# OpenDriveLab/ViDAR

Measured on AMD Instinct MI355X. Metric: train samples/sec (6-cam->BEV step), higher is better.
Workload: dtype f32

## Files before the change

vidar_amd/csrc/gemm_mfma.hip:

```cpp
#include <hip/hip_runtime.h>

#include <stdint.h>

#include <type_traits>

#include "vidar_hip.h"
#include "vidar_common.h"

namespace {

typedef __bf16 bf16x8 __attribute__((ext_vector_type(8)));
typedef __bf16 bf16x2 __attribute__((ext_vector_type(2)));
typedef float f32x16 __attribute__((ext_vector_type(16)));
typedef float f32x2 __attribute__((ext_vector_type(2)));
typedef float f32x4 __attribute__((ext_vector_type(4)));
typedef float f32x4u __attribute__((ext_vector_type(4), aligned(4)));
typedef uint32_t u32x4 __attribute__((ext_vector_type(4)));
typedef uint32_t u32x2 __attribute__((ext_vector_type(2)));

constexpr int BM = 128, BN = 128, THREADS = 256;
constexpr int BK = 32;
constexpr int MN_STRIDE = 128 + 8;
template <int PREC>
struct Geo {
  static constexpr int UNITS = (PREC == 1) ? 16 : 32;
  static constexpr int KM_STRIDE = (PREC == 1) ? UNITS : UNITS + 4;
  static constexpr int IMG_DWORDS = (128 * KM_STRIDE > UNITS * MN_STRIDE) ? 128 * KM_STRIDE : UNITS * MN_STRIDE;
  static constexpr int NS = UNITS / 8;
};
constexpr int PREC_F32 = 0, PREC_BF16X3 = 1;
constexpr int LAY_K = 0, LAY_MN = 1;

struct GemmArgs {
  const float* A; const float* B; float* C;
  int64_t lda, ldb, ldc, sA, sB, sC;
  int M, N, K;
  int splits, k_chunk;
  int slabs;
  const float* scale; const float* shift; int vec_axis;
  const float* residual; int64_t ldr, sR;
  int relu;
  int tiles_m, tiles_n, m_fastest;
  int total;
  float* a_rowsum;
  float* rowsum_ws;
};

struct Lane {
  int wm, wn, l31, h;
  __device__ __forceinline__ Lane(int tid, int wave) : wm((wave >> 1) * 64), wn((wave & 1) * 64), l31(tid & 31), h((tid & 63) >> 5) {}
  __device__ __forceinline__ explicit Lane(int tid) : Lane(tid, tid >> 6) {}
  __device__ __forceinline__ uint32_t voff(uint32_t ld) const { return (uint32_t)(((wm + 4 * h) * ld + wn + l31) * 4); }
};

__device__ __forceinline__ void zero_acc(f32x16 (&acc)[2][2]) {
#pragma unroll
  for (int i = 0; i < 2; ++i)
#pragma unroll
    for (int j = 0; j < 2; ++j)
#pragma unroll
      for (int r = 0; r < 16; ++r) acc[i][j][r] = 0.0f;
}

struct Staged {
  static constexpr int CH = 2;
  f32x4 v[CH][2];
};

constexpr int KM_LPR = 8;
constexpr int KM_RPI = 64 / KM_LPR;
constexpr int KM_NI = 32 / KM_RPI;

__device__ __forceinline__ __amdgpu_buffer_rsrc_t make_rsrc(const float* p, int64_t bytes = 0x7fffffff) {
  const uint64_t a = (uint64_t)p;
  const uint32_t lo = __builtin_amdgcn_readfirstlane((uint32_t)a), hi = __builtin_amdgcn_readfirstlane((uint32_t)(a >> 32));
  const int32_t n = __builtin_amdgcn_readfirstlane((int32_t)(bytes > 0x7fffffff ? 0x7fffffff : bytes));
  return __builtin_amdgcn_make_buffer_rsrc((void*)(((uint64_t)hi << 32) | lo), 0, n, 0x00020000);
}
__device__ __forceinline__ __amdgpu_buffer_rsrc_t window_rsrc(const float* base, int64_t ld, int rows_left, int cols_left,
                                                              bool present = true) {
  return make_rsrc(base, present ? ((int64_t)(rows_left - 1) * ld + cols_left) * 4 : 0);
}
__device__ __forceinline__ f32x4 ld16(__amdgpu_buffer_rsrc_t r, uint32_t voff, uint32_t soff) {
  return __builtin_bit_cast(f32x4, __builtin_amdgcn_raw_buffer_load_b128(r, voff, soff, 0));
}
__device__ __forceinline__ float ld4(__amdgpu_buffer_rsrc_t r, uint32_t voff, uint32_t soff) {
  return __builtin_bit_cast(float, __builtin_amdgcn_raw_buffer_load_b32(r, voff, soff, 0));
}

template <int PREC, int LAY>
__device__ __forceinline__ uint32_t voff(int64_t ld, int tid) {
  if (LAY == LAY_K) {
    const int lane = tid & 63, wave = tid >> 6;
    return (uint32_t)(((32 * wave + lane / KM_LPR) * (uint32_t)ld + (lane % KM_LPR) * 4) * 4);
  }
  const int kr = (PREC == PREC_BF16X3) ? (tid >> 5) * 2 : (tid >> 5);
  return (uint32_t)((kr * (uint32_t)ld + (tid & 31) * 4) * 4);
}

template <int PREC, int LAY>
__device__ __forceinline__ void load(Staged& s, __amdgpu_buffer_rsrc_t rs, int64_t ld, int krel, int k0, int kend, int tid,
                                     uint32_t vo) {
  if (LAY == LAY_K) {
#pragma unroll
    for (int i = 0; i < KM_NI; ++i)
      s.v[i >> 1][i & 1] = ld16(rs, vo, (uint32_t)((i * KM_RPI * (uint32_t)ld + krel) * 4));
    const bool tail = k0 + BK > kend;
    if (tail) {
      const int k = k0 + ((tid & 63) % KM_LPR) * 4;
#pragma unroll
      for (int i = 0; i < KM_NI; ++i)
#pragma unroll
        for (int j = 0; j < 4; ++j) s.v[i >> 1][i & 1][j] = (k + j < kend) ? s.v[i >> 1][i & 1][j] : 0.0f;
    }
  } else {
#pragma unroll
    for (int i = 0; i < Staged::CH * 2; ++i) {
      const int ku = (PREC == PREC_BF16X3) ? 16 * (i >> 1) + (i & 1) : 8 * i;
      s.v[i >> 1][i & 1] = ld16(rs, vo, (uint32_t)(krel + ku) * (uint32_t)ld * 4u);
    }
  }
}

__device__ __forceinline__ void split2(float a, float b, uint32_t& hi, uint32_t& lo) {
  f32x2 x = {a, b};
  bf16x2 h = __builtin_convertvector(x, bf16x2);
  f32x2 r = x - __builtin_convertvector(h, f32x2);
  bf16x2 l = __builtin_convertvector(r, bf16x2);
  hi = __builtin_bit_cast(uint32_t, h);
  lo = __builtin_bit_cast(uint32_t, l);
}

template <int PREC, int LAY>
__device__ __forceinline__ void stage(const Staged& s, uint32_t* img, int tid) {
  if (LAY == LAY_K) {
    const int lane = tid & 63, wave = tid >> 6;
    const int r0 = 32 * wave + lane / KM_LPR, kq = lane % KM_LPR;
#pragma unroll
    for (int i = 0; i < KM_NI; ++i) {
      const int r = r0 + i * KM_RPI;
      const f32x4 v = s.v[i >> 1][i & 1];
      if (PREC == PREC_BF16X3) {
        uint32_t h0, l0, h1, l1;
        split2(v[0], v[1], h0, l0);
        split2(v[2], v[3], h1, l1);
        const int pos = r * Geo<PREC>::KM_STRIDE + ((((kq >> 1) ^ ((r >> 2) & 3)) << 2) | ((kq & 1) << 1));
        *(u32x2*)(img + pos) = u32x2{h0, h1};
        *(u32x2*)(img + Geo<PREC>::IMG_DWORDS + pos) = u32x2{l0, l1};
      } else {
        *(u32x4*)(img + r * Geo<PREC>::KM_STRIDE + 4 * kq) = __builtin_bit_cast(u32x4, v);
      }
    }
  } else if (PREC == PREC_BF16X3) {
#pragma unroll
    for (int c = 0; c < 2; ++c) {
      const int item = tid + 256 * c;
      const int cq = (item & 31) * 4, u = item >> 5;
      u32x4 hi, lo;
#pragma unroll
      for (int j = 0; j < 4; ++j) {
        uint32_t h, l;
        split2(s.v[c][0][j], s.v[c][1][j], h, l);
        hi[j] = h; lo[j] = l;
      }
      *(u32x4*)(img + u * MN_STRIDE + cq) = hi;
      *(u32x4*)(img + Geo<PREC>::IMG_DWORDS + u * MN_STRIDE + cq) = lo;
    }
  } else {
#pragma unroll
    for (int i = 0; i < 4; ++i) {
      const int item = tid + 256 * i;
      *(u32x4*)(img + (item >> 5) * MN_STRIDE + (item & 31) * 4) = __builtin_bit_cast(u32x4, s.v[i >> 1][i & 1]);
    }
  }
}
template <int PREC, int ALAY, int BLAY>
__device__ __forceinline__ void stage_pair(const Staged& sa, const Staged& sb, uint32_t* imgA, uint32_t* imgB, int tid) {
  stage<PREC, ALAY>(sa, imgA, tid);
  stage<PREC, BLAY>(sb, imgB, tid);
}

template <int PREC, int LAY>
__device__ __forceinline__ u32x4 frag(const uint32_t* img, int row, int s, int h) {
  if (LAY == LAY_K) {
    if (PREC == PREC_BF16X3)
      return *(const u32x4*)(img + row * Geo<PREC>::KM_STRIDE + (((2 * s + h) ^ ((row >> 2) & 3)) << 2));
    return *(const u32x4*)(img + row * Geo<PREC>::KM_STRIDE + 8 * s + 4 * h);
  }
  u32x4 f;
  const uint32_t* p = img + (8 * s + 4 * h) * MN_STRIDE + row;
#pragma unroll
  for (int j = 0; j < 4; ++j) f[j] = p[j * MN_STRIDE];
  return f;
}

struct Tile {
  int z, batch, m0, n0, kbeg, kend;
  __amdgpu_buffer_rsrc_t rsA, rsB;
};

template <int PREC, int ALAY, int BLAY>
__device__ __forceinline__ Tile decode_tile(const GemmArgs& g, int t) {
  const int per_z = g.tiles_m * g.tiles_n;
  int id;
  {
    const int q = g.total >> 3, r = g.total & 7, x = t & 7;
    id = (x < r ? x * (q + 1) : r * (q + 1) + (x - r) * q) + (t >> 3);
  }
  Tile T;
  T.z = __builtin_amdgcn_readfirstlane(id / per_z);
  const int tt = id - T.z * per_z;
  const int tm = __builtin_amdgcn_readfirstlane(g.m_fastest ? tt % g.tiles_m : tt / g.tiles_n);
  const int tn = __builtin_amdgcn_readfirstlane(g.m_fastest ? tt / g.tiles_m : tt % g.tiles_n);
  T.batch = __builtin_amdgcn_readfirstlane(T.z / g.splits);
  const int split = T.z - T.batch * g.splits;
  T.m0 = tm * BM; T.n0 = tn * BN;
  T.kbeg = split * g.k_chunk;
  T.kend = min(g.K, T.kbeg + g.k_chunk);
  const float* A = g.A + (int64_t)T.batch * g.sA;
  const float* B = g.B + (int64_t)T.batch * g.sB;
  const int kleft = g.K - T.kbeg;
  T.rsA = ALAY == LAY_K ? window_rsrc(A + (int64_t)T.m0 * g.lda + T.kbeg, g.lda, g.M - T.m0, kleft)
                        : window_rsrc(A + (int64_t)T.kbeg * g.lda + T.m0, g.lda, kleft, g.M - T.m0);
  T.rsB = BLAY == LAY_K ? window_rsrc(B + (int64_t)T.n0 * g.ldb + T.kbeg, g.ldb, g.N - T.n0, kleft)
                        : window_rsrc(B + (int64_t)T.kbeg * g.ldb + T.n0, g.ldb, kleft, g.N - T.n0);
  return T;
}

template <int PREC, int ALAY, int BLAY>
__device__ __forceinline__ void fetch(Staged& sa, Staged& sb, const GemmArgs& g, const Tile& T, int k0, int tid, uint32_t voa,
                                      uint32_t vob) {
  load<PREC, ALAY>(sa, T.rsA, g.lda, k0 - T.kbeg, k0, T.kend, tid, voa);
  load<PREC, BLAY>(sb, T.rsB, g.ldb, k0 - T.kbeg, k0, T.kend, tid, vob);
}

__device__ __forceinline__ void add_rowsum(f32x4& rs, const Staged& sa) {
#pragma unroll
  for (int i = 0; i < Staged::CH * 2; ++i) rs += sa.v[i >> 1][i & 1];
}

template <int PREC, int ALAY, int BLAY>
__device__ __forceinline__ void mma_step(f32x16 (&acc)[2][2], const uint32_t* imgA, const uint32_t* imgB, const Lane& c) {
  constexpr int IMGS = (PREC == PREC_BF16X3) ? 2 : 1;
  constexpr int IMG_DWORDS = Geo<PREC>::IMG_DWORDS;
#pragma unroll
  for (int s = 0; s < Geo<PREC>::NS; ++s) {
    u32x4 fa[2][IMGS], fb[2][IMGS];
#pragma unroll
    for (int i = 0; i < 2; ++i)
#pragma unroll
      for (int p = 0; p < IMGS; ++p) {
        fa[i][p] = frag<PREC, ALAY>(imgA + p * IMG_DWORDS, c.wm + 32 * i + c.l31, s, c.h);
        fb[i][p] = frag<PREC, BLAY>(imgB + p * IMG_DWORDS, c.wn + 32 * i + c.l31, s, c.h);
      }
    if (PREC == PREC_BF16X3) {
#pragma unroll
      for (int term = 0; term < 3; ++term)
#pragma unroll
        for (int i = 0; i < 2; ++i)
#pragma unroll
          for (int j = 0; j < 2; ++j) {
            const bf16x8 a = __builtin_bit_cast(bf16x8, fa[i][term == 0 ? IMGS - 1 : 0]);
            const bf16x8 b = __builtin_bit_cast(bf16x8, fb[j][term == 1 ? IMGS - 1 : 0]);
            acc[i][j] = __builtin_amdgcn_mfma_f32_32x32x16_bf16(a, b, acc[i][j], 0, 0, 0);
          }
    } else {
#pragma unroll
      for (int u = 0; u < 4; ++u)
#pragma unroll
        for (int i = 0; i < 2; ++i)
#pragma unroll
          for (int j = 0; j < 2; ++j) {
            const f32x4 bf = __builtin_bit_cast(f32x4, fb[j][0]), af = __builtin_bit_cast(f32x4, fa[i][0]);
            acc[i][j] = __builtin_amdgcn_mfma_f32_32x32x2f32(af[u], bf[u], acc[i][j], 0, 0, 0);
          }
    }
  }
}

template <int PREC, int ALAY, int BLAY>
__device__ __forceinline__ void mainloop(f32x16 (&acc)[2][2], Staged& sa, Staged& sb, const GemmArgs& g, const Tile& T,
                                         int kstop, uint32_t* imgA, uint32_t* imgB, int tid, uint32_t voa, uint32_t vob,
                                         f32x4& rowsum, bool want_rowsum) {
  const Lane c(tid);
  for (int k0 = T.kbeg; k0 < kstop; k0 += BK) {
    if (ALAY == LAY_MN && want_rowsum) add_rowsum(rowsum, sa);
    stage_pair<PREC, ALAY, BLAY>(sa, sb, imgA, imgB, tid);
    __syncthreads();
    if (k0 + BK < T.kend) fetch<PREC, ALAY, BLAY>(sa, sb, g, T, k0 + BK, tid, voa, vob);
    mma_step<PREC, ALAY, BLAY>(acc, imgA, imgB, c);
    __syncthreads();
  }
}

__device__ __forceinline__ float finish(float acc, float sc, float sh, float rs, int relu) {
  float y = acc * sc + sh + rs;
  if (relu && !(y > 0.0f)) y = 0.0f;
  return y;
}

template <bool RAGGED_M>
__device__ __forceinline__ void epilogue_impl(const f32x16 (&acc)[2][2], const GemmArgs& g, const Tile& T, int tid) {
  const Lane c(tid);
  const int m0 = T.m0, n0 = T.n0;
  float* C; int64_t ldc;
  if (g.slabs) { C = g.C + (int64_t)T.z * g.M * g.N; ldc = g.N; }
  else { C = g.C + (int64_t)T.batch * g.sC; ldc = g.ldc; }
  const bool epi = !g.slabs;
  const bool by_n = epi && g.vec_axis == 0, by_m = epi && g.vec_axis == 1;
  const int rows_left = g.M - m0, cols_left = g.N - n0;
  const int mleft = rows_left - c.wm - 4 * c.h;
  const __amdgpu_buffer_rsrc_t rsC = window_rsrc(C + (int64_t)m0 * ldc + n0, ldc, rows_left, cols_left);
  const uint32_t voC = c.voff((uint32_t)ldc);
  const bool has_res = epi && g.residual != nullptr;
  const float* Rp = has_res ? g.residual + (int64_t)T.batch * g.sR + (int64_t)m0 * g.ldr + n0 : C;
  const __amdgpu_buffer_rsrc_t rsR = window_rsrc(Rp, g.ldr, rows_left, cols_left, has_res);
  const uint32_t voR = c.voff((uint32_t)g.ldr);
  const bool m_scale = by_m && g.scale != nullptr, m_shift = by_m && g.shift != nullptr;
  const __amdgpu_buffer_rsrc_t rsS = make_rsrc(m_scale ? g.scale + m0 : C, m_scale ? (int64_t)rows_left * 4 : 0);
  const __amdgpu_buffer_rsrc_t rsH = make_rsrc(m_shift ? g.shift + m0 : C, m_shift ? (int64_t)rows_left * 4 : 0);
  const uint32_t voM = (uint32_t)((c.wm + 4 * c.h) * 4);
#pragma unroll
  for (int j = 0; j < 2; ++j) {
    const int n = n0 + c.wn + 32 * j + c.l31;
    if (n >= g.N) continue;
    float sn = 1.0f, bn = 0.0f;
    if (by_n && g.scale) sn = g.scale[n];
    if (by_n && g.shift) bn = g.shift[n];
#pragma unroll
    for (int i = 0; i < 2; ++i) {
#pragma unroll
      for (int r0 = 0; r0 < 16; r0 += 8) {
        float sc[8], sh[8], rs[8];
#pragma unroll
        for (int r = 0; r < 8; ++r) {
          const int row = 32 * i + (r & 3) + 8 * ((r0 + r) >> 2);
          sc[r] = m_scale ? ld4(rsS, voM, (uint32_t)(row * 4)) : sn;
          sh[r] = m_shift ? ld4(rsH, voM, (uint32_t)(row * 4)) : bn;
          rs[r] = has_res ? ld4(rsR, voR, (uint32_t)((row * (uint32_t)g.ldr + 32 * j) * 4)) : 0.0f;
        }
#pragma unroll
        for (int r = 0; r < 8; ++r) {
          const int row = 32 * i + (r & 3) + 8 * ((r0 + r) >> 2);
          float y = acc[i][j][r0 + r];
          if (epi) y = finish(y, sc[r], sh[r], rs[r], g.relu);
          if (!RAGGED_M || row < mleft)
            __builtin_amdgcn_raw_buffer_store_b32(__builtin_bit_cast(uint32_t, y), rsC, voC,
                                                    (uint32_t)((row * (uint32_t)ldc + 32 * j) * 4), 0);
        }
      }
    }
  }
}

__device__ __forceinline__ void epilogue(const f32x16 (&acc)[2][2], const GemmArgs& g, const Tile& T, int tid) {
  if (g.M - T.m0 >= BM) epilogue_impl<false>(acc, g, T, tid);
  else epilogue_impl<true>(acc, g, T, tid);
}

constexpr int TAB_DWORDS = 2 * (BM + BM);

__device__ __forceinline__ void lds_barrier() { asm volatile("s_waitcnt lgkmcnt(0)\n\ts_barrier" ::: "memory"); }

__device__ __forceinline__ bool piped_tile(const GemmArgs& g, const Tile& T) {
  return !g.slabs && (g.vec_axis == 1 || (g.scale == nullptr && g.shift == nullptr)) && g.M - T.m0 >= BM &&
         g.N - T.n0 >= BN && T.kbeg < T.kend;
}

__device__ __forceinline__ float table_value(const GemmArgs& g, const Tile& T, int tid) {
  const float* v = tid < BM ? g.scale : g.shift;
  float x = tid < BM ? 1.0f : 0.0f;
  if (v != nullptr) x = v[T.m0 + (tid & (BM - 1))];
  return x;
}

template <int ALAY, int BLAY>
__device__ __forceinline__ void last_step_stage(const Staged& sa, const Staged& sb, uint32_t* imgA, uint32_t* imgB,
                                                float* tab, float tabv, int tid) {
  stage_pair<PREC_F32, ALAY, BLAY>(sa, sb, imgA, imgB, tid);
  tab[tid] = tabv;
  __syncthreads();
}

template <int ALAY, int BLAY>
__device__ __forceinline__ void last_step_piped(f32x16 (&acc)[2][2], const GemmArgs& g, const Tile& T, const uint32_t* imgA,
                                                const uint32_t* imgB, const float* tab, int tid0) {
  constexpr int PREC = PREC_F32;
  int tid = tid0;
  asm volatile("" : "+v"(tid));
  const Lane c(tid);
  const __amdgpu_buffer_rsrc_t rsC =
      window_rsrc(g.C + (int64_t)T.batch * g.sC + (int64_t)T.m0 * g.ldc + T.n0, g.ldc, BM, BN);
  const uint32_t ldc = (uint32_t)g.ldc, ldr = (uint32_t)g.ldr;
  const uint32_t voC = c.voff(ldc);
  const bool has_res = g.residual != nullptr;
  const __amdgpu_buffer_rsrc_t rsR = window_rsrc(
      has_res ? g.residual + (int64_t)T.batch * g.sR + (int64_t)T.m0 * g.ldr + T.n0 : g.C, g.ldr, BM, BN, has_res);
  const uint32_t voRz = has_res ? c.voff(ldr) : 0u;
  const uint32_t rb = has_res ? 4u : 0u;
  const float* tsc = tab + c.wm + 4 * c.h;
  const float* tsh = tsc + BM;
  float rs[16];
#pragma unroll
  for (int r = 0; r < 16; ++r) rs[r] = ld4(rsR, voRz, (uint32_t)((((r & 3) + 8 * (r >> 2)) * ldr) * rb));
  __builtin_amdgcn_sched_barrier(0);
#pragma unroll
  for (int sub = 0; sub <= 4; ++sub) {
    const int i = (sub >> 1) & 1, j = sub & 1;
    const int pi = ((sub - 1) >> 1) & 1, pj = (sub - 1) & 1;
    asm volatile("" ::: "memory");
#pragma unroll
    for (int s = 0; s < 4; ++s) {
      f32x4 af = {0.f, 0.f, 0.f, 0.f}, bf = af;
      if (sub < 4) {
        af = __builtin_bit_cast(f32x4, frag<PREC, ALAY>(imgA, c.wm + 32 * i + c.l31, s, c.h));
        bf = __builtin_bit_cast(f32x4, frag<PREC, BLAY>(imgB, c.wn + 32 * j + c.l31, s, c.h));
      }
#pragma unroll
      for (int u = 0; u < 4; ++u) {
        if (sub < 4) acc[i][j] = __builtin_amdgcn_mfma_f32_32x32x2f32(af[u], bf[u], acc[i][j], 0, 0, 0);
        if (sub > 0) {
          const int r = 4 * s + u;
          const int prow = 32 * pi + 8 * s + u;
          const float y = finish(acc[pi][pj][r], tsc[prow], tsh[prow], rs[r], g.relu);
          __builtin_amdgcn_raw_buffer_store_b32(__builtin_bit_cast(uint32_t, y), rsC, voC, (uint32_t)((prow * ldc + 32 * pj) * 4), 0);
          if (sub < 4) rs[r] = ld4(rsR, voRz, (uint32_t)(((32 * i + 8 * s + u) * ldr + 32 * j) * rb));
        }
      }
      __builtin_amdgcn_sched_barrier(0);
    }
    if (sub == 3) lds_barrier();
  }
}

template <int PREC, int ALAY, int BLAY>
__global__ __launch_bounds__(THREADS, 3) void gemm_mfma_kernel(GemmArgs g) {
  constexpr int IMGS = (PREC == PREC_BF16X3) ? 2 : 1;
  constexpr int IMGS_DWORDS = 2 * IMGS * Geo<PREC>::IMG_DWORDS;
  __shared__ __attribute__((aligned(16))) uint32_t lds[IMGS_DWORDS + (PREC == PREC_F32 && ALAY == LAY_K ? TAB_DWORDS : 0)];
  uint32_t* imgA = lds;
  uint32_t* imgB = lds + IMGS * Geo<PREC>::IMG_DWORDS;
  const int tid = threadIdx.x;
  const uint32_t voa = voff<PREC, ALAY>(g.lda, tid), vob = voff<PREC, BLAY>(g.ldb, tid);
  Staged sa, sb;
  int t = blockIdx.x;
  if (t >= g.total) return;
  Tile cur = decode_tile<PREC, ALAY, BLAY>(g, t);
  if (cur.kbeg < cur.kend) fetch<PREC, ALAY, BLAY>(sa, sb, g, cur, cur.kbeg, tid, voa, vob);
  for (int parity = 0;; parity ^= 1) {
    f32x16 acc[2][2];
    zero_acc(acc);
    f32x4 rowsum = {0.f, 0.f, 0.f, 0.f};
    const bool want_rowsum = ALAY == LAY_MN && g.a_rowsum != nullptr && cur.n0 == 0;
    const int tn = t + (int)gridDim.x;
    const bool more = tn < g.total;
    constexpr bool PIPED = PREC == PREC_F32 && ALAY == LAY_K;
    const bool piped = PIPED && piped_tile(g, cur);
    float tabv = 0.0f;
    if (piped) tabv = table_value(g, cur, tid);
    const int kstop = piped ? cur.kbeg + (cur.kend - cur.kbeg - 1) / BK * BK : cur.kend;
    mainloop<PREC, ALAY, BLAY>(acc, sa, sb, g, cur, kstop, imgA, imgB, tid, voa, vob, rowsum, want_rowsum);
    float* tab = reinterpret_cast<float*>(lds) + IMGS_DWORDS + parity * (TAB_DWORDS / 2);
    if constexpr (PIPED) {
      if (piped) last_step_stage<ALAY, BLAY>(sa, sb, imgA, imgB, tab, tabv, tid);
    }
    if (want_rowsum) {
      float* red = reinterpret_cast<float*>(lds);
      const int quad = tid & 31, part = tid >> 5;
      *(f32x4*)(red + (part * 32 + quad) * 4) = rowsum;
      __syncthreads();
      if (tid < BM) {
        float sum = 0.f;
#pragma unroll
        for (int p8 = 0; p8 < 8; ++p8) sum += red[(p8 * 32 + (tid >> 2)) * 4 + (tid & 3)];
        if (cur.m0 + tid < g.M) g.rowsum_ws[(int64_t)cur.z * g.M + cur.m0 + tid] = sum;
      }
      __syncthreads();
    }
    if (more) {
      const Tile nxt = decode_tile<PREC, ALAY, BLAY>(g, tn);
      if (nxt.kbeg < nxt.kend) fetch<PREC, ALAY, BLAY>(sa, sb, g, nxt, nxt.kbeg, tid, voa, vob);
    }
    if constexpr (PIPED) {
      if (piped) last_step_piped<ALAY, BLAY>(acc, g, cur, imgA, imgB, tab, tid);
      else epilogue(acc, g, cur, tid);
    } else {
      epilogue(acc, g, cur, tid);
    }
    if (!more) break;
    cur = decode_tile<PREC, ALAY, BLAY>(g, tn);
    t = tn;
  }
}

constexpr int WS_THREADS = 512;

template <int PREC, int ALAY, int BLAY>
struct Cursor {
  int t;
  int k0;
  Tile T;
  __device__ __forceinline__ void start(const GemmArgs& g, int t0) {
    t = t0;
    while (t < g.total) {
      T = decode_tile<PREC, ALAY, BLAY>(g, t);
      if (T.kbeg < T.kend) break;
      t += (int)gridDim.x;
    }
    k0 = (t < g.total) ? T.kbeg : 0;
  }
  __device__ __forceinline__ bool valid(const GemmArgs& g) const { return t < g.total; }
  __device__ __forceinline__ void advance(const GemmArgs& g) {
    k0 += BK;
    if (k0 >= T.kend) start(g, t + (int)gridDim.x);
  }
};

template <int PREC, int ALAY, int BLAY>
__global__ __launch_bounds__(WS_THREADS, 2) void gemm_mfma_ws_kernel(GemmArgs g) {
  constexpr int IMGS = (PREC == PREC_BF16X3) ? 2 : 1;
  constexpr int IMG_DWORDS = Geo<PREC>::IMG_DWORDS;
  constexpr int STAGE_DWORDS = 2 * IMGS * IMG_DWORDS;
  __shared__ __attribute__((aligned(16))) uint32_t lds[2 * STAGE_DWORDS];
  const int tid = threadIdx.x;
  const int wave = __builtin_amdgcn_readfirstlane(tid >> 6);
  if ((int)blockIdx.x >= g.total) return;

  if (wave >= 4) {
    const int ptid = tid - 256;
    const uint32_t voa = voff<PREC, ALAY>(g.lda, ptid), vob = voff<PREC, BLAY>(g.ldb, ptid);
    Staged sa0, sb0, sa1, sb1;
    Cursor<PREC, ALAY, BLAY> rd;
    rd.start(g, (int)blockIdx.x);
    int steps = 0;
    for (int t = (int)blockIdx.x; t < g.total; t += (int)gridDim.x) {
      const Tile T = decode_tile<PREC, ALAY, BLAY>(g, t);
      steps += (T.kend > T.kbeg) ? (T.kend - T.kbeg + BK - 1) / BK : 0;
    }
    const auto request = [&](Staged& sa, Staged& sb) {
      if (rd.valid(g)) { fetch<PREC, ALAY, BLAY>(sa, sb, g, rd.T, rd.k0, ptid, voa, vob); rd.advance(g); }
    };
    const auto produce = [&](Staged& sa, Staged& sb, int slot) {
      uint32_t* imgA = lds + slot * STAGE_DWORDS;
      stage_pair<PREC, ALAY, BLAY>(sa, sb, imgA, imgA + IMGS * IMG_DWORDS, ptid);
      request(sa, sb);
      lds_barrier();
    };
    request(sa0, sb0);
    request(sa1, sb1);
    for (int gs = 0; gs < steps; gs += 2) {
      produce(sa0, sb0, 0);
      if (gs + 1 < steps) produce(sa1, sb1, 1);
    }
    return;
  }

  const Lane c(tid, wave);
  int gs = 0;
  for (int t = (int)blockIdx.x; t < g.total; t += (int)gridDim.x) {
    const Tile T = decode_tile<PREC, ALAY, BLAY>(g, t);
    f32x16 acc[2][2];
    zero_acc(acc);
    for (int k0 = T.kbeg; k0 < T.kend; k0 += BK, ++gs) {
      lds_barrier();
      const uint32_t* imgA = lds + (gs & 1) * STAGE_DWORDS;
      mma_step<PREC, ALAY, BLAY>(acc, imgA, imgA + IMGS * IMG_DWORDS, c);
    }
    epilogue(acc, g, T, tid);
  }
}

__global__ __launch_bounds__(256) void gemm_slab_reduce_kernel(const float* __restrict__ ws, int Z, GemmArgs g) {
  __shared__ f32x4 part[4][64];
  if (g.a_rowsum != nullptr) {
    const int lane = threadIdx.x & 63;
    for (int m = (int)blockIdx.x * 4 + (threadIdx.x >> 6); m < g.M; m += (int)gridDim.x * 4) {
      float a = 0.f;
      for (int z = lane; z < Z; z += 64) a += g.rowsum_ws[(int64_t)z * g.M + m];
#pragma unroll
      for (int off = 32; off > 0; off >>= 1) a += __shfl_xor(a, off, 64);
      if (lane == 0) g.a_rowsum[m] = a;
    }
  }
  const int64_t total = (int64_t)g.M * g.N;
  const int64_t quads = total >> 2;
  const int col = threadIdx.x & 63, zg = threadIdx.x >> 6;
  for (int64_t q0 = (int64_t)blockIdx.x * 64; q0 < quads + 1; q0 += (int64_t)gridDim.x * 64) {
    const int64_t q = q0 + col;
    f32x4 a = {0.f, 0.f, 0.f, 0.f};
    if (q < quads) {
      for (int z = zg; z < Z; z += 4) a += *(const f32x4u*)(ws + (int64_t)z * total + 4 * q);
    } else if (q == quads) {
      for (int z = zg; z < Z; z += 4)
        for (int e = 0; e < (int)(total & 3); ++e) a[e] += ws[(int64_t)z * total + 4 * q + e];
    }
    part[zg][col] = a;
    __syncthreads();
    if (zg == 0 && q <= quads) {
      const f32x4 sum = ((part[0][col] + part[1][col]) + part[2][col]) + part[3][col];
      const int n_el = q < quads ? 4 : (int)(total & 3);
      for (int e = 0; e < n_el; ++e) {
        const int64_t idx = 4 * q + e;
        const int m = (int)(idx / g.N), n = (int)(idx - (int64_t)m * g.N);
        const int vi = g.vec_axis == 1 ? m : n;
        g.C[(int64_t)m * g.ldc + n] = finish(sum[e], g.scale ? g.scale[vi] : 1.0f, g.shift ? g.shift[vi] : 0.0f,
                                             g.residual ? g.residual[(int64_t)m * g.ldr + n] : 0.0f, g.relu);
      }
    }
    __syncthreads();
  }
}

int g_gemm_variant = 0;

template <class F>
void with_layouts(int a_layout, int b_layout, F f) {
  using K = std::integral_constant<int, LAY_K>;
  using MN = std::integral_constant<int, LAY_MN>;
  if (a_layout == LAY_K && b_layout == LAY_K) f(K{}, K{});
  else if (a_layout == LAY_K) f(K{}, MN{});
  else if (b_layout == LAY_K) f(MN{}, K{});
  else f(MN{}, MN{});
}

template <int PREC>
void launch(const GemmArgs& g, int a_layout, int b_layout, bool ws, int grid, hipStream_t st) {
  with_layouts(a_layout, b_layout, [&](auto a, auto b) {
    constexpr int ALAY = decltype(a)::value, BLAY = decltype(b)::value;
    if (ws) hipLaunchKernelGGL((gemm_mfma_ws_kernel<PREC, ALAY, BLAY>), dim3(grid), dim3(WS_THREADS), 0, st, g);
    else hipLaunchKernelGGL((gemm_mfma_kernel<PREC, ALAY, BLAY>), dim3(grid), dim3(THREADS), 0, st, g);
  });
}

int num_cus() {
  static int cached[64] = {0};
  int dev = 0;
  if (hipGetDevice(&dev) != hipSuccess || dev < 0 || dev >= 64) return 256;
  if (cached[dev] == 0) {
    hipDeviceProp_t prop;
    cached[dev] = (hipGetDeviceProperties(&prop, dev) == hipSuccess && prop.multiProcessorCount > 0)
                      ? prop.multiProcessorCount : 256;
  }
  return cached[dev];
}

int pick_splits(int M, int N, int K, int batch) {
  const int tiles = ((M + BM - 1) / BM) * ((N + BN - 1) / BN) * batch;
  int s = (512 + tiles - 1) / tiles;
  const int max_s = (K + 4 * BK - 1) / (4 * BK);
  if (s > max_s) s = max_s;
  if (s < 1) s = 1;
  if (s > 256) s = 256;
  return s;
}

size_t slab_workspace_bytes(int Z, int M, int N, bool rowsum) {
  return (size_t)Z * ((size_t)M * N + (rowsum ? M : 0)) * sizeof(float);
}

int resident_grid(int total, int per_cu) {
  const int resident = num_cus() * per_cu / 8 * 8;
  return total > resident ? resident : total;
}

}

extern "C" {

int vidar_gemm_set_variant(int variant) {
  const int prev = g_gemm_variant;
  g_gemm_variant = (variant < 0 || variant > 2) ? 0 : variant;
  return prev;
}

int vidar_gemm_splits(int M, int N, int K, int batch, int precision, int reduce) {
  if (!reduce) return 1;
  return pick_splits(M, N, K, batch);
}

size_t vidar_gemm_workspace_bytes(int M, int N, int K, int batch, int precision, int reduce) {
  if (!reduce) return 0;
  const int Z = batch * pick_splits(M, N, K, batch);
  if (reduce == 1) return Z > 1 ? slab_workspace_bytes(Z, M, N, false) : 0;
  return slab_workspace_bytes(Z, M, N, true);
}

int vidar_gemm_f32(const float* A, int64_t lda, int a_layout, const float* B, int64_t ldb, int b_layout, float* C,
                   int64_t ldc, int M, int N, int K, int batch, int64_t strideA, int64_t strideB, int64_t strideC,
                   const float* scale, const float* shift, int vec_axis, const float* residual, int64_t ldr,
                   int64_t strideR, int relu, int precision, int reduce, float* a_rowsum, void* workspace,
                   size_t workspace_bytes, void* stream) {
  VIDAR_ENTER();
  if (a_rowsum != nullptr && !(reduce && a_layout == LAY_MN)) return VIDAR_ERR_BAD_ARG;
  if (A == nullptr || B == nullptr || C == nullptr || M <= 0 || N <= 0 || K <= 0 || batch <= 0) return VIDAR_ERR_BAD_ARG;
  if ((a_layout != LAY_K && a_layout != LAY_MN) || (b_layout != LAY_K && b_layout != LAY_MN)) return VIDAR_ERR_BAD_ARG;
  if (precision != PREC_F32 && precision != PREC_BF16X3) return VIDAR_ERR_BAD_ARG;
  if (vec_axis != 0 && vec_axis != 1) return VIDAR_ERR_BAD_ARG;
  if (lda < (a_layout == LAY_K ? K : M) || ldb < (b_layout == LAY_K ? K : N) || ldc < N) return VIDAR_ERR_BAD_ARG;
  if (residual != nullptr && (ldr < N || ldr >= (1 << 22))) return VIDAR_ERR_BAD_ARG;
  if (ldc >= (1 << 22)) return VIDAR_ERR_BAD_ARG;
  if (lda >= (1 << 22) || ldb >= (1 << 22)) return VIDAR_ERR_BAD_ARG;
  if ((a_layout == LAY_MN && (int64_t)K * lda >= (1LL << 29)) || (b_layout == LAY_MN && (int64_t)K * ldb >= (1LL << 29)))
    return VIDAR_ERR_BAD_ARG;
  hipStream_t st = (hipStream_t)stream;
  GemmArgs g;
  g.A = A; g.B = B; g.C = C;
  g.lda = lda; g.ldb = ldb; g.ldc = ldc; g.sA = strideA; g.sB = strideB; g.sC = strideC;
  g.M = M; g.N = N; g.K = K;
  g.scale = scale; g.shift = shift; g.vec_axis = vec_axis; g.residual = residual; g.ldr = ldr; g.sR = strideR;
  g.relu = relu;
  g.tiles_m = (M + BM - 1) / BM; g.tiles_n = (N + BN - 1) / BN;
  g.m_fastest = M < N;
  g.splits = reduce ? pick_splits(M, N, K, batch) : 1;
  g.k_chunk = ((K + g.splits - 1) / g.splits + BK - 1) / BK * BK;
  const int Z = batch * g.splits;
  g.slabs = (reduce && (Z > 1 || a_rowsum != nullptr)) ? 1 : 0;
  g.a_rowsum = a_rowsum;
  g.rowsum_ws = nullptr;
  if ((int64_t)g.tiles_m * g.tiles_n * Z > 0x3fffffff) return VIDAR_ERR_BAD_ARG;
  g.total = g.tiles_m * g.tiles_n * Z;
  if (reduce && (strideC != 0 || strideR != 0) && batch > 1) return VIDAR_ERR_BAD_ARG;
  if (g.slabs) {
    if (workspace == nullptr || workspace_bytes < slab_workspace_bytes(Z, M, N, a_rowsum != nullptr)) return VIDAR_ERR_BAD_ARG;
    g.rowsum_ws = a_rowsum ? (float*)workspace + (size_t)Z * M * N : nullptr;
  }
  const bool ws = g_gemm_variant >= 1 && a_rowsum == nullptr;
  const int grid = resident_grid(g.total, ws ? g_gemm_variant : 3);
  GemmArgs tiles = g;
  if (g.slabs) tiles.C = (float*)workspace;
  if (precision == PREC_BF16X3) launch<PREC_BF16X3>(tiles, a_layout, b_layout, ws, grid, st);
  else launch<PREC_F32>(tiles, a_layout, b_layout, ws, grid, st);
  if (g.slabs) {
    const int64_t total = (int64_t)M * N;
    int blocks = (int)((total / 4 + 1 + 63) / 64);
    if (blocks > 4096) blocks = 4096;
    hipLaunchKernelGGL(gemm_slab_reduce_kernel, dim3(blocks), dim3(256), 0, st, (const float*)workspace, Z, g);
  }
  return vidar_last_error();
}

}
```

vidar_amd/gemm.py:

```python
from __future__ import annotations

import contextlib
import os

import torch

from ._lib import lib, check, ptr, stream_of, workspace, TIMER
from . import deterministic

F32, BF16X3 = 0, 1
K_MAJOR, MN_MAJOR = 0, 1
_MODES = ("lib", "auto", "f32", "bf16x3")
_mode = os.environ.get("VIDAR_GEMM", "auto")
if _mode not in _MODES:
    raise ValueError(f"VIDAR_GEMM={_mode!r}: expected one of {_MODES}")


def mode() -> str:
    return _mode


def set_mode(m: str) -> str:
    global _mode
    if m not in _MODES:
        raise ValueError(f"gemm mode {m!r}: expected one of {_MODES}")
    prev, _mode = _mode, m
    return prev


@contextlib.contextmanager
def use(m: str):
    prev = set_mode(m)
    try:
        yield
    finally:
        set_mode(prev)


def precision_of(m: str | None = None) -> int:
    m = _mode if m is None else m
    return BF16X3 if m == "bf16x3" else F32


def own_kernels(m: str | None = None) -> bool:
    return (_mode if m is None else m) in ("f32", "bf16x3")


def _f32c(t, what):
    if not t.is_cuda:
        raise RuntimeError(f"vidar_gemm: {what} must be a CUDA tensor (no CPU path)")
    if t.dtype != torch.float32:
        raise TypeError(f"vidar_gemm: {what} must be float32, got {t.dtype}")
    if t.dim() and t.stride(-1) != 1:
        raise ValueError(f"vidar_gemm: the last dimension of {what} must be contiguous (strides {tuple(t.stride())})")
    return t


_LD_MAX = 1 << 22
_KLD_MAX = 1 << 29


def operand_ok(t, layout, contraction) -> bool:
    if not (t.is_cuda and t.dtype == torch.float32 and t.dim() >= 2 and t.stride(-1) == 1):
        return False
    ld = t.stride(-2)
    if ld < t.shape[-1] or ld >= _LD_MAX:
        return False
    return layout == K_MAJOR or contraction * ld < _KLD_MAX


def _operand(t, layout, contraction, what):
    if not t.is_cuda:
        raise RuntimeError(f"vidar_gemm: {what} must be a CUDA tensor (no CPU path)")
    if t.dtype != torch.float32:
        raise TypeError(f"vidar_gemm: {what} must be float32, got {t.dtype}")
    if operand_ok(t, layout, contraction):
        return t
    c = t.contiguous()
    if not operand_ok(c, layout, contraction):
        raise ValueError(f"vidar_gemm: {what} {tuple(t.shape)} exceeds the kernel's addressing range "
                         f"(leading dimension < 2^22, contraction x leading dimension < 2^29)")
    return c


def gemm_raw(A, lda, a_layout, B, ldb, b_layout, C, ldc, M, N, K, *, batch=1, sA=0, sB=0, sC=0, scale=None, shift=None,
             vec_axis=0, residual=None, ldr=0, sR=0, relu=False, precision=F32, reduce=False, a_rowsum=None, name="gemm"):
    L = lib()
    ws, ws_ptr, nbytes = workspace(L.vidar_gemm_workspace_bytes, M, N, K, batch, precision, 2 if a_rowsum is not None else 1,
                                   like=C) if reduce else (None, None, 0)
    flops = 2.0 * M * N * K * batch
    with TIMER.span(name, flops):
        check(L.vidar_gemm_f32(ptr(A), lda, a_layout, ptr(B), ldb, b_layout, ptr(C), ldc, M, N, K, batch, sA, sB, sC,
                               ptr(scale), ptr(shift), vec_axis, ptr(residual), ldr, sR, bool(relu), precision,
                               bool(reduce), ptr(a_rowsum), ws_ptr, nbytes, stream_of(C)),
              "vidar_gemm_f32")
    return C


def linear_forward(x2, weight, bias=None, relu=False, precision=F32):
    M, K = x2.shape
    N = weight.shape[0]
    x2 = _operand(x2, K_MAJOR, K, "x"); weight = _operand(weight, K_MAJOR, K, "weight")
    y = torch.empty((M, N), dtype=torch.float32, device=x2.device)
    if M == 0:
        return y
    return gemm_raw(x2, x2.stride(0), K_MAJOR, weight, weight.stride(0), K_MAJOR, y, N, M, N, K,
                    shift=None if bias is None else _f32c(bias, "bias"), vec_axis=0, relu=relu, precision=precision,
                    name="gemm_linear_fwd")


def linear_grad_input(g2, weight, precision=F32):
    M, N = g2.shape
    K = weight.shape[1]
    g2 = _operand(g2, K_MAJOR, N, "grad_out"); weight = _operand(weight, MN_MAJOR, N, "weight")
    gx = torch.empty((M, K), dtype=torch.float32, device=g2.device)
    if M == 0:
        return gx
    return gemm_raw(g2, g2.stride(0), K_MAJOR, weight, weight.stride(0), MN_MAJOR, gx, K, M, K, N, precision=precision,
                    name="gemm_linear_dx")


def linear_grad_weight(g2, x2, precision=F32, with_bias=False):
    M, N = g2.shape
    K = x2.shape[1]
    g2 = _operand(g2, MN_MAJOR, M, "grad_out"); x2 = _operand(x2, MN_MAJOR, M, "x")
    gw = torch.empty((N, K), dtype=torch.float32, device=g2.device)
    gb = torch.empty(N, dtype=torch.float32, device=g2.device) if with_bias else None
    if M == 0:
        return (gw.zero_(), gb.zero_()) if with_bias else gw.zero_()
    gemm_raw(g2, g2.stride(0), MN_MAJOR, x2, x2.stride(0), MN_MAJOR, gw, K, N, K, M, precision=precision,
             reduce=True, a_rowsum=gb, name="gemm_linear_dw")
    return (gw, gb) if with_bias else gw


def linear_grad_weight_ok(g2, x2) -> bool:
    return g2.dim() == 2 and x2.dim() == 2 and operand_ok(g2, MN_MAJOR, g2.shape[0]) and operand_ok(x2, MN_MAJOR, x2.shape[0])


def _colsum(g2):
    n = g2.shape[1]
    if deterministic.enabled():
        return g2.sum(0)
    if n % 4 == 0 and (n // 4) & (n // 4 - 1) == 0 and n <= 4096 and g2.data_ptr() % 16 == 0 and g2.is_contiguous():
        gb = torch.empty(n, dtype=torch.float32, device=g2.device)
        check(lib().vidar_colsum_f32(ptr(g2), ptr(gb), g2.shape[0], n, stream_of(g2)), "colsum")
        return gb
    return g2.sum(0)


class MfmaLinear(torch.autograd.Function):

    @staticmethod
    def forward(ctx, x2, weight, bias, relu, precision):
        x2 = x2 if x2.stride(-1) == 1 else x2.contiguous()
        weight = weight if weight.stride(-1) == 1 else weight.contiguous()
        y = linear_forward(x2, weight, bias, relu, precision)
        ctx.save_for_backward(x2, weight, y if relu else None)
        ctx.cfg = (relu, precision, bias is not None)
        return y

    @staticmethod
    @torch.autograd.function.once_differentiable
    def backward(ctx, g):
        x2, weight, y = ctx.saved_tensors
        relu, precision, has_bias = ctx.cfg
        g2 = g if (g.stride(-1) == 1 and g.dtype == torch.float32) else g.float().contiguous()
        if relu:
            g2 = g2 * (y > 0)
        gx = linear_grad_input(g2, weight, precision) if ctx.needs_input_grad[0] else None
        want_b = has_bias and ctx.needs_input_grad[2]
        gw = gb = None
        if ctx.needs_input_grad[1]:
            gw = linear_grad_weight(g2, x2, precision, with_bias=want_b)
            if want_b:
                gw, gb = gw
        elif want_b:
            gb = _colsum(g2)
        return gx, gw, gb, None, None


def linear(x, weight, bias=None, relu=False, m: str | None = None):
    n = weight.shape[0]
    y = MfmaLinear.apply(x.reshape(-1, x.shape[-1]), weight, bias, bool(relu), precision_of(m))
    return y.view(*x.shape[:-1], n)


def conv_forward(w2, x3, scale=None, shift=None, residual=None, relu=False, precision=F32):
    _f32c(w2, "weight"); _f32c(x3, "x")
    Bn, Ci, HW = x3.shape
    Co = w2.shape[0]
    y = torch.empty((Bn, Co, HW), dtype=torch.float32, device=x3.device)
    if residual is not None:
        assert residual.shape == y.shape and residual.is_contiguous()
    return gemm_raw(w2, w2.stride(0), K_MAJOR, x3, x3.stride(1), MN_MAJOR, y, HW, Co, HW, Ci, batch=Bn, sA=0,
                    sB=x3.stride(0), sC=Co * HW, scale=scale, shift=shift, vec_axis=1, residual=residual, ldr=HW,
                    sR=Co * HW, relu=relu, precision=precision, name="gemm_conv_fwd")


def conv_grad_input(w2, g3, precision=F32):
    _f32c(w2, "weight"); _f32c(g3, "grad_out")
    Bn, Co, HW = g3.shape
    Ci = w2.shape[1]
    gx = torch.empty((Bn, Ci, HW), dtype=torch.float32, device=g3.device)
    return gemm_raw(w2, w2.stride(0), MN_MAJOR, g3, g3.stride(1), MN_MAJOR, gx, HW, Ci, HW, Co, batch=Bn, sA=0,
                    sB=g3.stride(0), sC=Ci * HW, precision=precision, name="gemm_conv_dx")


def conv_grad_weight(g3, x3, precision=F32, scale=None):
    _f32c(g3, "grad_out"); _f32c(x3, "x")
    Bn, Co, HW = g3.shape
    Ci = x3.shape[1]
    gw = torch.empty((Co, Ci), dtype=torch.float32, device=g3.device)
    return gemm_raw(g3, g3.stride(1), K_MAJOR, x3, x3.stride(1), K_MAJOR, gw, Ci, Co, Ci, HW, batch=Bn,
                    sA=g3.stride(0), sB=x3.stride(0), scale=scale, vec_axis=1, precision=precision, reduce=True,
                    name="gemm_conv_dw")
```

Before: 2.952.

## Split ragged last-wave GEMM tiles along K with atomic-ticket reduction

Adds a planner that chooses split-K counts to cut down quantized-wave waste for reduce GEMMs. For non-reduce GEMMs whose tile count leaves a partial last wave, it cuts only the leftover tiles along K. The partial sums go to a workspace, and the last arriving block, chosen by an atomic ticket, sums the slabs and runs the epilogue. This aims to fill idle CUs in the tail wave. The cost is an extra memset, workspace traffic, and atomics and fences on those tiles.

```diff
diff --git a/vidar_amd/csrc/gemm_mfma.hip b/vidar_amd/csrc/gemm_mfma.hip
--- a/vidar_amd/csrc/gemm_mfma.hip
+++ b/vidar_amd/csrc/gemm_mfma.hip
@@ -6,6 +6,7 @@
 
 #include "vidar_hip.h"
 #include "vidar_common.h"
+#include "gemm_plan.h"
 
 namespace {
 
@@ -35,7 +36,8 @@
   const float* A; const float* B; float* C;
   int64_t lda, ldb, ldc, sA, sB, sC;
   int M, N, K;
-  int splits, k_chunk;
+  gemm_plan::Plan plan;
+  float* cut_ws;
   int slabs;
   const float* scale; const float* shift; int vec_axis;
   const float* residual; int64_t ldr, sR;
@@ -196,27 +198,25 @@
 
 struct Tile {
   int z, batch, m0, n0, kbeg, kend;
+  int cut_id;
   __amdgpu_buffer_rsrc_t rsA, rsB;
 };
 
 template <int PREC, int ALAY, int BLAY>
 __device__ __forceinline__ Tile decode_tile(const GemmArgs& g, int t) {
-  const int per_z = g.tiles_m * g.tiles_n;
-  int id;
-  {
-    const int q = g.total >> 3, r = g.total & 7, x = t & 7;
-    id = (x < r ? x * (q + 1) : r * (q + 1) + (x - r) * q) + (t >> 3);
-  }
+  const int per_z = g.plan.per_z;
+  const gemm_plan::Unit u = gemm_plan::unit_of(g.plan, g.K, t);
+  const int id = u.item;
   Tile T;
   T.z = __builtin_amdgcn_readfirstlane(id / per_z);
   const int tt = id - T.z * per_z;
   const int tm = __builtin_amdgcn_readfirstlane(g.m_fastest ? tt % g.tiles_m : tt / g.tiles_n);
   const int tn = __builtin_amdgcn_readfirstlane(g.m_fastest ? tt / g.tiles_m : tt % g.tiles_n);
-  T.batch = __builtin_amdgcn_readfirstlane(T.z / g.splits);
-  const int split = T.z - T.batch * g.splits;
+  T.batch = __builtin_amdgcn_readfirstlane(T.z / g.plan.splits);
   T.m0 = tm * BM; T.n0 = tn * BN;
-  T.kbeg = split * g.k_chunk;
-  T.kend = min(g.K, T.kbeg + g.k_chunk);
+  T.kbeg = __builtin_amdgcn_readfirstlane(u.kbeg);
+  T.kend = __builtin_amdgcn_readfirstlane(u.kend);
+  T.cut_id = __builtin_amdgcn_readfirstlane(u.cut_id);
   const float* A = g.A + (int64_t)T.batch * g.sA;
   const float* B = g.B + (int64_t)T.batch * g.sB;
   const int kleft = g.K - T.kbeg;
@@ -358,6 +358,71 @@
   else epilogue_impl<true>(acc, g, T, tid);
 }
 
+template <bool WG>
+__device__ __forceinline__ bool cut_collect(f32x16 (&acc)[2][2], const GemmArgs& g, const Tile& T, int tid0, uint32_t* lds) {
+  int tid = tid0;
+  asm volatile("" : "+v"(tid));
+  const Lane c(tid);
+  const int parts = g.plan.cut;
+  int* const cnt = reinterpret_cast<int*>(g.cut_ws + (int64_t)(g.plan.total - g.plan.whole) * (BM * BN));
+  const int tile = __builtin_amdgcn_readfirstlane(T.cut_id / parts);
+  const uint32_t vo = c.voff(BN);
+  {
+    const __amdgpu_buffer_rsrc_t rs = make_rsrc(g.cut_ws + (int64_t)T.cut_id * (BM * BN), BM * BN * 4);
+#pragma unroll
+    for (int i = 0; i < 2; ++i)
+#pragma unroll
+      for (int j = 0; j < 2; ++j)
+#pragma unroll
+        for (int r = 0; r < 16; ++r) {
+          const float y = acc[i][j][r];
+          __builtin_amdgcn_raw_buffer_store_b32(__builtin_bit_cast(uint32_t, y), rs, vo,
+                                                  (uint32_t)(((32 * i + (r & 3) + 8 * (r >> 2)) * BN + 32 * j) * 4), 0);
+        }
+  }
+  asm volatile("s_waitcnt vmcnt(0)" ::: "memory");
+  int ticket = 0;
+  if (WG) {
+    __syncthreads();
+    if (tid == 0) {
+      __builtin_amdgcn_fence(__ATOMIC_RELEASE, "agent");
+      asm volatile("s_waitcnt vmcnt(0)" ::: "memory");
+      lds[0] = (uint32_t)__hip_atomic_fetch_add(cnt + 4 * tile, 1, __ATOMIC_RELAXED, __HIP_MEMORY_SCOPE_AGENT);
+    }
+    __syncthreads();
+    ticket = (int)lds[0];
+    __syncthreads();
+  } else {
+    if ((tid & 63) == 0) {
+      __builtin_amdgcn_fence(__ATOMIC_RELEASE, "agent");
+      asm volatile("s_waitcnt vmcnt(0)" ::: "memory");
+      ticket = __hip_atomic_fetch_add(cnt + 4 * tile + (tid >> 6), 1, __ATOMIC_RELAXED, __HIP_MEMORY_SCOPE_AGENT);
+    }
+    ticket = __builtin_amdgcn_readfirstlane(ticket);
+  }
+  if (ticket != parts - 1) return false;
+  if (WG ? tid == 0 : (tid & 63) == 0) {
+    __builtin_amdgcn_fence(__ATOMIC_ACQUIRE, "agent");
+    asm volatile("s_waitcnt vmcnt(0)" ::: "memory");
+  }
+  if (WG) __syncthreads();
+  zero_acc(acc);
+  const __amdgpu_buffer_rsrc_t rs = make_rsrc(g.cut_ws + (int64_t)tile * parts * (BM * BN), (int64_t)parts * (BM * BN * 4));
+  for (uint32_t slab = 0; slab < (uint32_t)parts * (BM * BN * 4); slab += BM * BN * 4) {
+#pragma unroll
+    for (int i = 0; i < 2; ++i)
+#pragma unroll
+      for (int j = 0; j < 2; ++j) {
+        float v[16];
+#pragma unroll
+        for (int r = 0; r < 16; ++r) v[r] = ld4(rs, vo, slab + (uint32_t)(((32 * i + (r & 3) + 8 * (r >> 2)) * BN + 32 * j) * 4));
+#pragma unroll
+        for (int r = 0; r < 16; ++r) acc[i][j][r] += v[r];
+      }
+  }
+  return true;
+}
+
 constexpr int TAB_DWORDS = 2 * (BM + BM);
 
 __device__ __forceinline__ void lds_barrier() { asm volatile("s_waitcnt lgkmcnt(0)\n\ts_barrier" ::: "memory"); }
@@ -442,18 +507,18 @@
   uint32_t* imgB = lds + IMGS * Geo<PREC>::IMG_DWORDS;
   const int tid = threadIdx.x;
   const uint32_t voa = voff<PREC, ALAY>(g.lda, tid), vob = voff<PREC, BLAY>(g.ldb, tid);
+  const int wave = __builtin_amdgcn_readfirstlane(tid >> 6);
   Staged sa, sb;
   int t = blockIdx.x;
-  if (t >= g.total) return;
-  Tile cur = decode_tile<PREC, ALAY, BLAY>(g, t);
-  if (cur.kbeg < cur.kend) fetch<PREC, ALAY, BLAY>(sa, sb, g, cur, cur.kbeg, tid, voa, vob);
-  for (int parity = 0;; parity ^= 1) {
+  Tile cur = decode_tile<PREC, ALAY, BLAY>(g, t < g.plan.whole ? t : 0);
+  if (t < g.plan.whole && cur.kbeg < cur.kend) fetch<PREC, ALAY, BLAY>(sa, sb, g, cur, cur.kbeg, tid, voa, vob);
+  for (int parity = 0; t < g.plan.whole; parity ^= 1) {
     f32x16 acc[2][2];
     zero_acc(acc);
     f32x4 rowsum = {0.f, 0.f, 0.f, 0.f};
     const bool want_rowsum = ALAY == LAY_MN && g.a_rowsum != nullptr && cur.n0 == 0;
     const int tn = t + (int)gridDim.x;
-    const bool more = tn < g.total;
+    const bool more = tn < g.plan.whole;
     constexpr bool PIPED = PREC == PREC_F32 && ALAY == LAY_K;
     const bool piped = PIPED && piped_tile(g, cur);
     float tabv = 0.0f;
@@ -487,9 +552,23 @@
     } else {
       epilogue(acc, g, cur, tid);
     }
+    t = tn;
     if (!more) break;
     cur = decode_tile<PREC, ALAY, BLAY>(g, tn);
-    t = tn;
+  }
+  if (t >= g.total) return;
+  const int tid1 = wave * 64 + (int)__builtin_amdgcn_mbcnt_hi(~0u, __builtin_amdgcn_mbcnt_lo(~0u, 0u));
+  auto argp = __builtin_amdgcn_kernarg_segment_ptr();
+  asm volatile("" : "+s"(argp));
+  const GemmArgs& h = *(const GemmArgs*)argp;
+  for (; t < h.total; t += (int)gridDim.x) {
+    const Tile T = decode_tile<PREC, ALAY, BLAY>(h, t);
+    fetch<PREC, ALAY, BLAY>(sa, sb, h, T, T.kbeg, tid1, voa, vob);
+    f32x16 acc[2][2];
+    zero_acc(acc);
+    f32x4 rowsum = {0.f, 0.f, 0.f, 0.f};
+    mainloop<PREC, ALAY, BLAY>(acc, sa, sb, h, T, T.kend, imgA, imgB, tid1, voa, vob, rowsum, false);
+    if (cut_collect<true>(acc, h, T, tid1, lds)) epilogue_impl<true>(acc, h, T, tid1);
   }
 }
 
@@ -566,6 +645,7 @@
       const uint32_t* imgA = lds + (gs & 1) * STAGE_DWORDS;
       mma_step<PREC, ALAY, BLAY>(acc, imgA, imgA + IMGS * IMG_DWORDS, c);
     }
+    if (T.cut_id >= 0 && !cut_collect<false>(acc, g, T, tid, lds)) continue;
     epilogue(acc, g, T, tid);
   }
 }
@@ -644,14 +724,10 @@
   return cached[dev];
 }
 
-int pick_splits(int M, int N, int K, int batch) {
-  const int tiles = ((M + BM - 1) / BM) * ((N + BN - 1) / BN) * batch;
-  int s = (512 + tiles - 1) / tiles;
-  const int max_s = (K + 4 * BK - 1) / (4 * BK);
-  if (s > max_s) s = max_s;
-  if (s < 1) s = 1;
-  if (s > 256) s = 256;
-  return s;
+static_assert(gemm_plan::TILE == BM && gemm_plan::TILE == BN && gemm_plan::KSTEP == BK, "gemm_plan.h describes this kernel's tiles");
+
+gemm_plan::Plan plan_of(int M, int N, int K, int batch, bool reduce) {
+  return gemm_plan::make_plan((M + BM - 1) / BM, (N + BN - 1) / BN, batch, K, reduce, gemm_plan::residency(num_cus(), 3));
 }
 
 size_t slab_workspace_bytes(int Z, int M, int N, bool rowsum) {
@@ -659,7 +735,7 @@
 }
 
 int resident_grid(int total, int per_cu) {
-  const int resident = num_cus() * per_cu / 8 * 8;
+  const int resident = gemm_plan::residency(num_cus(), per_cu);
   return total > resident ? resident : total;
 }
 
@@ -674,13 +750,14 @@
 }
 
 int vidar_gemm_splits(int M, int N, int K, int batch, int precision, int reduce) {
-  if (!reduce) return 1;
-  return pick_splits(M, N, K, batch);
+  if (!reduce || M <= 0 || N <= 0 || K <= 0 || batch <= 0) return 1;
+  return plan_of(M, N, K, batch, true).splits;
 }
 
 size_t vidar_gemm_workspace_bytes(int M, int N, int K, int batch, int precision, int reduce) {
-  if (!reduce) return 0;
-  const int Z = batch * pick_splits(M, N, K, batch);
+  if (M <= 0 || N <= 0 || K <= 0 || batch <= 0) return 0;
+  if (!reduce) return gemm_plan::cut_workspace_bytes(plan_of(M, N, K, batch, false));
+  const int Z = batch * plan_of(M, N, K, batch, true).splits;
   if (reduce == 1) return Z > 1 ? slab_workspace_bytes(Z, M, N, false) : 0;
   return slab_workspace_bytes(Z, M, N, true);
 }
@@ -711,18 +788,23 @@
   g.relu = relu;
   g.tiles_m = (M + BM - 1) / BM; g.tiles_n = (N + BN - 1) / BN;
   g.m_fastest = M < N;
-  g.splits = reduce ? pick_splits(M, N, K, batch) : 1;
-  g.k_chunk = ((K + g.splits - 1) / g.splits + BK - 1) / BK * BK;
-  const int Z = batch * g.splits;
+  if ((int64_t)g.tiles_m * g.tiles_n * batch > 0x3fffffff / gemm_plan::MAX_PARTS) return VIDAR_ERR_BAD_ARG;
+  g.plan = plan_of(M, N, K, batch, reduce != 0);
+  const int Z = batch * g.plan.splits;
   g.slabs = (reduce && (Z > 1 || a_rowsum != nullptr)) ? 1 : 0;
   g.a_rowsum = a_rowsum;
   g.rowsum_ws = nullptr;
-  if ((int64_t)g.tiles_m * g.tiles_n * Z > 0x3fffffff) return VIDAR_ERR_BAD_ARG;
-  g.total = g.tiles_m * g.tiles_n * Z;
+  g.total = g.plan.total;
+  g.cut_ws = nullptr;
   if (reduce && (strideC != 0 || strideR != 0) && batch > 1) return VIDAR_ERR_BAD_ARG;
   if (g.slabs) {
     if (workspace == nullptr || workspace_bytes < slab_workspace_bytes(Z, M, N, a_rowsum != nullptr)) return VIDAR_ERR_BAD_ARG;
     g.rowsum_ws = a_rowsum ? (float*)workspace + (size_t)Z * M * N : nullptr;
+  }
+  if (g.plan.cut > 1) {
+    if (workspace == nullptr || workspace_bytes < gemm_plan::cut_workspace_bytes(g.plan)) return VIDAR_ERR_BAD_ARG;
+    g.cut_ws = (float*)workspace;
+    if (hipMemsetAsync((char*)workspace + gemm_plan::cut_slab_bytes(g.plan), 0, (size_t)g.plan.cut_tiles * 4 * sizeof(int), st) != hipSuccess) return vidar_last_error();
   }
   const bool ws = g_gemm_variant >= 1 && a_rowsum == nullptr;
   const int grid = resident_grid(g.total, ws ? g_gemm_variant : 3);
diff --git a/vidar_amd/csrc/gemm_plan.h b/vidar_amd/csrc/gemm_plan.h
--- /dev/null
+++ b/vidar_amd/csrc/gemm_plan.h
@@ -0,0 +1,141 @@
+#pragma once
+
+#include <stdint.h>
+
+#if defined(__HIPCC__)
+#define GEMM_PLAN_FN __host__ __device__ inline
+#else
+#define GEMM_PLAN_FN inline
+#endif
+
+namespace gemm_plan {
+
+constexpr int TILE = 128;
+constexpr int KSTEP = 32;
+constexpr int MIN_STEPS = 4;
+constexpr int MAX_PARTS = 256;
+
+inline int residency(int cus, int per_cu) {
+  const int r = cus * per_cu / 8 * 8;
+  return r < 8 ? 8 : r;
+}
+inline int round_of(int resident) {
+  const int p = resident / 3 / 8 * 8;
+  return p < 8 ? 8 : p;
+}
+
+struct Plan {
+  int per_z;
+  int splits, k_chunk;
+  int whole;
+  int cut, cut_chunk;
+  int cut_tiles;
+  int total;
+};
+
+struct Unit {
+  int item;
+  int kbeg, kend;
+  int cut_id;
+};
+
+inline int steps_of(int K) { return (K + KSTEP - 1) / KSTEP; }
+inline int chunk_of(int K, int parts) { return ((K + parts - 1) / parts + KSTEP - 1) / KSTEP * KSTEP; }
+inline int64_t rounds_of(int64_t units, int round) { return (units + round - 1) / round; }
+
+inline int base_splits(int64_t items, int K) {
+  int64_t s = (512 + items - 1) / items;
+  const int max_s = (K + MIN_STEPS * KSTEP - 1) / (MIN_STEPS * KSTEP);
+  if (s > max_s) s = max_s;
+  if (s < 1) s = 1;
+  if (s > MAX_PARTS) s = MAX_PARTS;
+  return (int)s;
+}
+
+inline bool ragged(int64_t units, int round) {
+  const int64_t tail = units % round;
+  return units > round && tail != 0 && tail * 10 < (int64_t)round * 9;
+}
+
+inline Plan make_plan(int tiles_m, int tiles_n, int batch, int K, bool reduce, int resident) {
+  Plan p;
+  p.per_z = tiles_m * tiles_n;
+  const int64_t items = (int64_t)p.per_z * batch;
+  const int round = round_of(resident);
+  p.splits = 1;
+  p.cut = 1; p.cut_chunk = 0; p.cut_tiles = 0;
+  if (reduce) {
+    const int s0 = base_splits(items, K);
+    int best = s0;
+    if (ragged(items * s0, round)) {
+      const int max_s = (K + MIN_STEPS * KSTEP - 1) / (MIN_STEPS * KSTEP);
+      int hi = 2 * s0;
+      if (hi > max_s) hi = max_s;
+      if (hi > MAX_PARTS) hi = MAX_PARTS;
+      int64_t best_cost = rounds_of(items * s0, round) * (chunk_of(K, s0) / KSTEP + 1);
+      for (int s = (s0 + 1) / 2; s <= hi; ++s) {
+        const int64_t cost = rounds_of(items * s, round) * (chunk_of(K, s) / KSTEP + 1);
+        if (cost < best_cost || (cost == best_cost && s < best)) { best_cost = cost; best = s; }
+      }
+    }
+    p.splits = best;
+  }
+  p.k_chunk = chunk_of(K, p.splits);
+  const int64_t units = items * p.splits;
+  p.whole = (int)units;
+  if (!reduce && ragged(items, round)) {
+    const int ksteps = steps_of(K);
+    const int64_t left = items % round;
+    int max_s = ksteps / MIN_STEPS;
+    if (max_s > MAX_PARTS) max_s = MAX_PARTS;
+    int best = 1;
+    int64_t best_cost = ksteps;
+    for (int s = 2; s <= max_s; ++s) {
+      const int cs = (ksteps + s - 1) / s;
+      if ((int64_t)(s - 1) * cs >= ksteps) continue;
+      const int64_t cost = rounds_of(left * s, round) * (cs + 1) + (s + 3) / 4;
+      if (cost < best_cost) { best_cost = cost; best = s; }
+    }
+    const int64_t before = (items / round + 1) * ksteps, after = (items / round) * ksteps + best_cost;
+    if (best > 1 && (before - after) * 20 >= before) {
+      p.cut = best;
+      p.cut_chunk = (ksteps + best - 1) / best * KSTEP;
+      p.cut_tiles = (int)left;
+      p.whole = (int)(items - left);
+    }
+  }
+  p.total = p.whole + p.cut_tiles * p.cut;
+  return p;
+}
+
+GEMM_PLAN_FN int xcd_order(int t, int total) {
+  const int q = total >> 3, r = total & 7, x = t & 7;
+  return (x < r ? x * (q + 1) : r * (q + 1) + (x - r) * q) + (t >> 3);
+}
+
+GEMM_PLAN_FN Unit unit_of(const Plan& p, int K, int t) {
+  Unit u;
+  int chunk, part;
+  if (t < p.whole) {
+    u.item = xcd_order(t, p.whole);
+    u.cut_id = -1;
+    part = (u.item / p.per_z) % p.splits;
+    chunk = p.k_chunk;
+  } else {
+    u.cut_id = xcd_order(t - p.whole, p.total - p.whole);
+    const int tile = u.cut_id / p.cut;
+    u.item = p.whole + tile;
+    part = u.cut_id - tile * p.cut;
+    chunk = p.cut_chunk;
+  }
+  u.kbeg = part * chunk;
+  u.kend = u.kbeg + chunk < K ? u.kbeg + chunk : K;
+  return u;
+}
+
+inline size_t cut_slab_bytes(const Plan& p) { return (size_t)p.cut_tiles * p.cut * TILE * TILE * sizeof(float); }
+inline size_t cut_workspace_bytes(const Plan& p) {
+  return p.cut > 1 ? cut_slab_bytes(p) + (size_t)p.cut_tiles * 4 * sizeof(int) : 0;
+}
+
+}
diff --git a/vidar_amd/gemm.py b/vidar_amd/gemm.py
--- a/vidar_amd/gemm.py
+++ b/vidar_amd/gemm.py
@@ -86,8 +86,8 @@
 def gemm_raw(A, lda, a_layout, B, ldb, b_layout, C, ldc, M, N, K, *, batch=1, sA=0, sB=0, sC=0, scale=None, shift=None,
              vec_axis=0, residual=None, ldr=0, sR=0, relu=False, precision=F32, reduce=False, a_rowsum=None, name="gemm"):
     L = lib()
-    ws, ws_ptr, nbytes = workspace(L.vidar_gemm_workspace_bytes, M, N, K, batch, precision, 2 if a_rowsum is not None else 1,
-                                   like=C) if reduce else (None, None, 0)
+    ws, ws_ptr, nbytes = workspace(L.vidar_gemm_workspace_bytes, M, N, K, batch, precision,
+                                   (2 if a_rowsum is not None else 1) if reduce else 0, like=C)
     flops = 2.0 * M * N * K * batch
     with TIMER.span(name, flops):
         check(L.vidar_gemm_f32(ptr(A), lda, a_layout, ptr(B), ldb, b_layout, ptr(C), ldc, M, N, K, batch, sA, sB, sC,
```

Measured after the change: 2.965 (median of 6 runs). About the same (+0.5%).
